# moxime/joint-vae

Measured on NVIDIA B200. Metric: train_images_per_sec, higher is better.
Workload: dtype bf16

## Files before the change

joint-vae_b200/csrc/conv.cu:

```cuda
#include "tc_common.cuh"
#include <vector>
#include <algorithm>
#include <stdlib.h>

namespace jvae {

constexpr int CONV_THREADS = 192;
constexpr int CONV_MAX_TAPS = 64;
static thread_local int g_last_conv_kernel = 0;

struct ConvParams {
  int N, Hq, Wq;
  int TW, TH, NB;
  int tiles_x, tiles_y, tiles_n, num_tiles, n_tiles_n;
  int Cblk, nCk, ntaps;
  int in_stride;
  short dy[CONV_MAX_TAPS], dx[CONV_MAX_TAPS];
  int BN;
  int Ho, Wo, Cout, ldc;
  int out_sy, out_sx, out_oy, out_ox;
  int act;
  int out_f32;
  const float* bias;
  __nv_bfloat16* out;
// ... 747 lines not shown
        int m = tile;
        const int tx = m % p.tiles_x; m /= p.tiles_x;
        const int ty = m % p.tiles_y; m /= p.tiles_y;
        const int n0 = m * p.NB;
        for (int t = 0; t < ntap; ++t, ++it) {
          const int s = it % p.stages;
          const uint32_t ph = (it / p.stages) & 1;
          mbar_wait(&empty_bar[s], ph ^ 1);
          uint8_t* sa = smem + (size_t)s * p.stage_bytes;
          mbar_arrive_expect_tx(&full_bar[s], p.tx_bytes);
          tma_load_4d(sa, &tmap_dy, &full_bar[s], cy0, tx * p.TW, ty * p.TH, n0);
          tma_load_4d(sa + p.a_bytes, &tmap_x, &full_bar[s], cx0, tx * p.TW * p.in_stride + p.dx[tap_lo + t],
                      ty * p.TH * p.in_stride + p.dy[tap_lo + t], n0);
        }
      }
    }
  } else if (warp == 1) {
    if (elect_one()) {
      const uint32_t idesc = make_idesc_bf16(64, p.Cblk_x, true, true);
      const uint32_t swz_y = (p.Cblk_y == 64) ? SWZ_128B : (p.Cblk_y == 32 ? SWZ_64B : SWZ_32B);
      const uint32_t swz_x = (p.Cblk_x == 64) ? SWZ_128B : (p.Cblk_x == 32 ? SWZ_64B : SWZ_32B);
      const uint32_t row_y = (uint32_t)p.Cblk_y * 2u, row_x = (uint32_t)p.Cblk_x * 2u;
      uint32_t it = 0;
      bool first_tile = true;
      for (int tile = blockIdx.x; tile < p.num_tiles; tile += gridDim.x) {
        for (int t = 0; t < ntap; ++t, ++it) {
          const int s = it % p.stages;
          const uint32_t ph = (it / p.stages) & 1;
          mbar_wait(&full_bar[s], ph);
          tc_fence_after();
          const uint32_t sa = smem_u32(smem + (size_t)s * p.stage_bytes);
          const uint64_t a_desc = make_smem_desc(sa, 8 * row_y, 8 * row_y, swz_y);
          const uint64_t b_desc = make_smem_desc(sa + p.a_bytes, 8 * row_x, 8 * row_x, swz_x);
          const uint32_t d_tmem = tmem_base + (uint32_t)(t * p.Cblk_x);
#pragma unroll
          for (int k = 0; k < 8; ++k)
            umma_bf16(d_tmem, a_desc + (uint64_t)((16 * row_y * k) >> 4), b_desc + (uint64_t)((16 * row_x * k) >> 4), idesc,
                      (!first_tile || k != 0));
          umma_commit(&empty_bar[s]);
        }
        first_tile = false;
      }
      umma_commit(done_bar);
    }
  } else {
    const int q = warp & 3;
    mbar_wait(done_bar, 0);
    tc_fence_after();
    const bool has_work = blockIdx.x < p.num_tiles;
    for (int t = 0; t < ntap && has_work; ++t) {
      for (int c0 = 0; c0 < p.Cblk_x; c0 += 16) {
        uint32_t r[16];
        tmem_ld_32x16(tmem_base + ((uint32_t)(q * 32) << 16) + (uint32_t)(t * p.Cblk_x + c0), r);
        tmem_ld_wait();
        const int row = q * 16 + lane;
        if (lane < 16 && row < M_real) {
          float* o = p.dw + (size_t)(tap_lo + t) * p.dw_ld_tap + (size_t)(cy0 + row) * p.dw_ld_co + (size_t)(cx0 + c0) * p.dw_ld_cx;
#pragma unroll
          for (int j = 0; j < 16; ++j)
            if (c0 + j < N_real) atomicAdd(o + (size_t)j * p.dw_ld_cx, __uint_as_float(r[j]));
        }
      }
    }
  }
  tc_fence_before();
  __syncthreads();
  if (warp == 1) tmem_dealloc_dyn(tmem_base, p.tmem_cols);
}

constexpr int WH_MAX_GROUPS = 64;
struct WHaloParams {
  int N, Hq, Wq;
  int NBt, HHs, HWp, MT, strips_x, num_boxes;
  int RT, blocks_y;
  uint32_t g_img_bytes;
  int Cblk_g, Cblk_x, ncx, Cg, Cx;
  int ngroups, groups_per_cta;
  int dymin, dxmin, ey;
  int in_stride, nplanes;
  short plane_ry[4], plane_rx[4];
  uint32_t plane_bytes;
  uint32_t grp_off16[WH_MAX_GROUPS];
  unsigned char grp_ntap[WH_MAX_GROUPS];
  unsigned char grp_nv[WH_MAX_GROUPS];
  uint32_t grp_boff16[WH_MAX_GROUPS];
  uint32_t grp_idesc[WH_MAX_GROUPS];
  unsigned short grp_col[WH_MAX_GROUPS];
  short grp_tap[WH_MAX_GROUPS][8][8];
  uint32_t g_gap_bytes;
  float* dw;
  int dw_ld_tap, dw_ld_co, dw_ld_cx;
  uint32_t x_stage_bytes, stage_bytes, x_box_bytes, g_box_bytes, tmem_cols;
  int stages;
};

__global__ void __launch_bounds__(CONV_THREADS, 1)
conv_wgrad_halo_kernel(const __grid_constant__ CUtensorMap tmap_g, const __grid_constant__ CUtensorMap tmap_x,
                       const __grid_constant__ WHaloParams p) {
  extern __shared__ uint8_t smem_raw[];
  uint8_t* smem = reinterpret_cast<uint8_t*>((reinterpret_cast<uintptr_t>(smem_raw) + 1023) & ~(uintptr_t)1023);
  uint64_t* full_bar = reinterpret_cast<uint64_t*>(smem + (size_t)p.stages * p.stage_bytes);
  uint64_t* empty_bar = full_bar + 8;
  uint64_t* done_bar = empty_bar + 8;
  uint32_t* tmem_slot = reinterpret_cast<uint32_t*>(done_bar + 1);
  const int warp = threadIdx.x >> 5, lane = threadIdx.x & 31;
  const int g_lo = (int)blockIdx.y * p.groups_per_cta;
  const int ng = min(p.groups_per_cta, p.ngroups - g_lo);
  const int cg0 = ((int)blockIdx.z / p.ncx) * p.Cblk_g, cx0 = ((int)blockIdx.z % p.ncx) * p.Cblk_x;
  const uint32_t rbx = (uint32_t)p.Cblk_x * 2u, rbg = (uint32_t)p.Cblk_g * 2u;

  for (uint32_t i = threadIdx.x; i < (uint32_t)p.stages * p.stage_bytes / 16u; i += CONV_THREADS)
    reinterpret_cast<uint4*>(smem)[i] = make_uint4(0u, 0u, 0u, 0u);
  if (warp == 0 && lane == 0) {
    tma_prefetch_desc(&tmap_g);
    tma_prefetch_desc(&tmap_x);
    for (int s = 0; s < 8; ++s) { mbar_init(&full_bar[s], 1); mbar_init(&empty_bar[s], 1); }
    mbar_init(done_bar, 1);
    fence_barrier_init();
  }
  fence_proxy_async();
  if (warp == 1) tmem_alloc_dyn(tmem_slot, p.tmem_cols);
  tc_fence_before();
  __syncthreads();
  tc_fence_after();
  const uint32_t tmem_base = *tmem_slot;

  if (warp == 0) {
    if (elect_one()) {
      uint32_t s = 0, ph = 0;
      for (int box = blockIdx.x; box < p.num_boxes; box += gridDim.x) {
        int m = box;
        const int sx = m % p.strips_x; m /= p.strips_x;
        const int by = m % p.blocks_y; const int nb = m / p.blocks_y;
        mbar_wait(&empty_bar[s], ph ^ 1);
        uint8_t* st = smem + (size_t)s * p.stage_bytes;
        mbar_arrive_expect_tx(&full_bar[s], p.x_box_bytes + p.g_box_bytes);
        for (int pl = 0; pl < p.nplanes; ++pl)
          tma_load_4d(st + (size_t)pl * p.plane_bytes, &tmap_x, &full_bar[s], cx0, p.in_stride * (sx * 8 + p.dxmin) + p.plane_rx[pl],
                      p.in_stride * (by * p.RT + p.dymin) + p.plane_ry[pl], nb * p.NBt);
        if (p.blocks_y == 1) {
          tma_load_4d(st + p.x_stage_bytes + p.g_gap_bytes, &tmap_g, &full_bar[s], cg0, sx * 8, 0, nb * p.NBt);
        } else {
          for (int i = 0; i < p.NBt; ++i)
            tma_load_4d(st + p.x_stage_bytes + p.g_gap_bytes + (size_t)i * p.HHs * 8u * rbg, &tmap_g, &full_bar[s], cg0, sx * 8,
                        by * p.RT, nb * p.NBt + i);
        }
        if (++s == (uint32_t)p.stages) { s = 0; ph ^= 1; }
      }
    }
  } else if (warp == 1) {
    if (elect_one()) {
      const uint32_t swx = (p.Cblk_x == 64) ? SWZ_128B : (p.Cblk_x == 32 ? SWZ_64B : SWZ_32B);
      const uint32_t swg = (p.Cblk_g == 64) ? SWZ_128B : (p.Cblk_g == 32 ? SWZ_64B : SWZ_32B);
      const uint32_t a_hi = (((uint32_t)p.HWp * rbx >> 4) & 0x3fffu) | (1u << 14) | (swx << 29);
      const uint32_t b_hi = (((8u * rbg) >> 4) & 0x3fffu) | (1u << 14) | (swg << 29);
      const uint32_t a_lbo = ((rbx >> 4) & 0x3fffu) << 16, b_lbo = (((8u * rbg) >> 4) & 0x3fffu) << 16;
      const uint32_t ak16 = (2u * (uint32_t)p.HWp * rbx) >> 4, bk16 = (16u * rbg) >> 4;
      const uint32_t am16 = (16u * (uint32_t)p.HWp * rbx) >> 4, bm16 = (128u * rbg) >> 4;
      const uint32_t ey_slots16 = ((uint32_t)p.ey * 8u * rbg) >> 4;
      uint32_t s = 0, ph = 0, first = 0;
      for (int box = blockIdx.x; box < p.num_boxes; box += gridDim.x) {
        mbar_wait(&full_bar[s], ph);
        tc_fence_after();
        const uint32_t sx_ = smem_u32(smem + (size_t)s * p.stage_bytes);
        const uint32_t a_lo0 = ((sx_ >> 4) & 0x3fffu) | a_lbo;
        const uint32_t b_lo0 = ((((sx_ + p.x_stage_bytes + p.g_gap_bytes) >> 4) - ey_slots16) & 0x3fffu) | b_lbo;
        for (int m = 0; m < p.MT; ++m) {
          const uint32_t b_lo = b_lo0 + (uint32_t)m * bm16;
          for (int g = 0; g < ng; ++g) {
            const uint32_t a_lo = a_lo0 + (uint32_t)m * am16 + p.grp_off16[g_lo + g];
            const uint32_t bg_lo = b_lo + p.grp_boff16[g_lo + g];
            const uint32_t idesc = p.grp_idesc[g_lo + g];
            const uint32_t d = tmem_base + (uint32_t)p.grp_col[g_lo + g];
#pragma unroll
            for (int k = 0; k < 8; ++k)
              umma_bf16(d, desc64(a_hi, a_lo + (uint32_t)k * ak16), desc64(b_hi, bg_lo + (uint32_t)k * bk16), idesc,
                        k == 0 ? first : 1u);
          }
          first = 1;
        }
        umma_commit(&empty_bar[s]);
        if (++s == (uint32_t)p.stages) { s = 0; ph ^= 1; }
      }
      umma_commit(done_bar);
    }
  } else {
    const int q = warp & 3;
    mbar_wait(done_bar, 0);
    tc_fence_after();
    const bool has_work = (int)blockIdx.x < p.num_boxes;
    const int Ng = min(p.Cblk_g, p.Cg - cg0), Nx = min(p.Cblk_x, p.Cx - cx0);
    for (int g = 0; g < ng && has_work; ++g) {
      const int ntap = p.grp_ntap[g_lo + g];
      const bool m128 = ntap * p.Cblk_x > 64;
      const int row = m128 ? q * 32 + lane : q * 16 + lane;
      const bool row_ok = m128 || lane < 16;
      const int j = row / p.Cblk_x, cx = row - j * p.Cblk_x;
      const bool live = row_ok && j < ntap && cx < Nx;
      const int nv = p.grp_nv[g_lo + g];
      for (int jv = 0; jv < nv; ++jv) {
        const int t = live ? p.grp_tap[g_lo + g][jv][j] : 0;
        for (int c0 = 0; c0 < p.Cblk_g; c0 += 16) {
          uint32_t r[16];
          tmem_ld_32x16(tmem_base + ((uint32_t)(q * 32) << 16) + (uint32_t)(p.grp_col[g_lo + g] + jv * p.Cblk_g + c0), r);
          tmem_ld_wait();
          if (live) {
            float* o = p.dw + (size_t)t * p.dw_ld_tap + (size_t)(cg0 + c0) * p.dw_ld_co + (size_t)(cx0 + cx) * p.dw_ld_cx;
#pragma unroll
            for (int i = 0; i < 16; ++i)
              if (c0 + i < Ng) atomicAdd(o + (size_t)i * p.dw_ld_co, __uint_as_float(r[i]));
          }
        }
      }
    }
  }
  tc_fence_before();
  __syncthreads();
  if (warp == 1) tmem_dealloc_dyn(tmem_base, p.tmem_cols);
}

static int pow2_floor(int v) { int p = 1; while (p * 2 <= v) p *= 2; return p; }
static int pow2_ceil(int v) { int p = 1; while (p < v) p *= 2; return p; }

static void tile_shape(int Hq, int Wq, int* TW, int* TH, int* NB) {
  int tw = pow2_floor(Wq); if (tw > 128) tw = 128;
  if (tw < Wq && tw * 2 <= 128 && (tw * 2 - Wq) * 4 <= Wq) tw *= 2;
  int th = pow2_ceil(Hq); if (th > 128 / tw) th = 128 / tw;
  *TW = tw; *TH = th; *NB = 128 / (tw * th);
}

static int cblk_of(int C) { return C > 32 ? 64 : (C > 16 ? 32 : 16); }

static int act_tmap(CUtensorMap* t, const void* base, int N, int H, int W, int C, int ldc, int Cblk, int TW, int TH, int NB,
                    int stride) {
  uint64_t dims[4] = {(uint64_t)C, (uint64_t)W, (uint64_t)H, (uint64_t)N};
  uint64_t strides[3] = {(uint64_t)ldc * 2, (uint64_t)W * ldc * 2, (uint64_t)H * W * ldc * 2};
  uint32_t box[4] = {(uint32_t)Cblk, (uint32_t)(TW * stride), (uint32_t)(TH * stride), (uint32_t)NB};
  uint32_t es[4] = {1, (uint32_t)stride, (uint32_t)stride, 1};
  return make_tmap_bf16(t, base, 4, dims, strides, box, es, Cblk * 2);
}

struct PhaseSpec { int n; const int16_t* ntaps; const int16_t* oy; const int16_t* ox; };

static int try_launch_halo(const void* in, int N, int H, int W, int Cin, int ld_in, const void* wmat, int Cout_pad, int ldw,
                           int ntaps, const int16_t* tap_dy, const int16_t* tap_dx, int in_stride, int Hq, int Wq, void* out,
                           int Ho, int Wo, int Cout, int ld_out, int out_sy, int out_sx, int out_oy, int out_ox,
                           const float* bias, int act, double* stats, const jvae_bn_reduce* bn, int* bn_fused,
                           cudaStream_t stream, const PhaseSpec* phs = nullptr, HaloParams* plan_out = nullptr,
                           int force_cblk = 0, double* score_out = nullptr) {
  if (Wq < 6) return 1;
  const bool wide = Cin > 64 || Cout_pad > 64;
  if (phs && (wide || in_stride != 1 || phs->n < 2 || phs->n > 4 || bn)) return 1;
  if (wide) {
    const bool wide_on = getenv("JVAE_CONV_WIDE") && atoi(getenv("JVAE_CONV_WIDE")) != 0;
    if (!wide_on || (Cout_pad > 64 && (Cout_pad % 64) != 0) || bn) return 1;
  }
  if (bn && !(out_sy == 1 && out_sx == 1 && out_oy == 0 && out_ox == 0 && Ho == Hq && Wo == Wq)) {
    bn = nullptr; stats = nullptr;
  }
  if (!phs && !wide && force_cblk == 0 && Cin > 32 && !(getenv("JVAE_CONV_KSPLIT") && atoi(getenv("JVAE_CONV_KSPLIT")) == 0)) {
    HaloParams pa, pb;
    double sa = 0.0, sb = 0.0;
    const int ra = try_launch_halo(in, N, H, W, Cin, ld_in, wmat, Cout_pad, ldw, ntaps, tap_dy, tap_dx, in_stride, Hq, Wq, out, Ho, Wo,
                                   Cout, ld_out, out_sy, out_sx, out_oy, out_ox, bias, act, stats, bn, nullptr, stream, nullptr, &pa, 64, &sa);
    const int rb2 = try_launch_halo(in, N, H, W, Cin, ld_in, wmat, Cout_pad, ldw, ntaps, tap_dy, tap_dx, in_stride, Hq, Wq, out, Ho, Wo,
                                    Cout, ld_out, out_sy, out_sx, out_oy, out_ox, bias, act, stats, bn, nullptr, stream, nullptr, &pb, 32, &sb);
    if (ra < 0) return ra;
    const int pick = (rb2 == 0 && (ra != 0 || sb > 1.15 * sa)) ? 32 : 64;
    if (score_out) *score_out = pick == 32 ? sb : sa;
    return try_launch_halo(in, N, H, W, Cin, ld_in, wmat, Cout_pad, ldw, ntaps, tap_dy, tap_dx, in_stride, Hq, Wq, out, Ho, Wo, Cout,
                           ld_out, out_sy, out_sx, out_oy, out_ox, bias, act, stats, bn, bn_fused, stream, nullptr, plan_out, pick, nullptr);
  }
  HaloParams p;
  memset(&p, 0, sizeof(p));
  p.PH = 1;
  const int st = in_stride;
  int tey[CONV_MAX_TAPS], tex[CONV_MAX_TAPS], tpl[CONV_MAX_TAPS];
  int dymin = 1 << 20, dymax = -(1 << 20), dxmin = 1 << 20, dxmax = -(1 << 20);
  p.in_stride = st; p.nplanes = 0;
  for (int t = 0; t < ntaps; ++t) {
    p.dy[t] = tap_dy[t]; p.dx[t] = tap_dx[t];
    const int ry = ((tap_dy[t] % st) + st) % st, rx = ((tap_dx[t] % st) + st) % st;
    tey[t] = (tap_dy[t] - ry) / st; tex[t] = (tap_dx[t] - rx) / st;
    int pl = -1;
    for (int i = 0; i < p.nplanes; ++i)
      if (p.plane_ry[i] == ry && p.plane_rx[i] == rx) pl = i;
    if (pl < 0) { pl = p.nplanes++; p.plane_ry[pl] = (short)ry; p.plane_rx[pl] = (short)rx; }
    tpl[t] = pl;
    dymin = min(dymin, tey[t]); dymax = max(dymax, tey[t]);
// ... 194 lines not shown
      p.ck[nck].y = ((uint32_t)(col_base[ci] + q.e_hi - (u - j0)) * p.w_tap_bytes) >> 4;
      p.ck[nck].z = make_idesc_bf16(128, (j1 - j0 + 1) * p.BN, false, false);
      p.ck[nck].w = (uint32_t)(j0 * p.BN) | (fresh ? 0x80000000u : 0u);
      ++nck;
    };
    std::vector<int> fresh_u;
    for (int jn = 0; jn < p.G;) {
      const int u = jn + cols[0].e_hi;
      fresh_u.push_back(u);
      jn = min(p.G - 1, u - cols[0].e_lo) + 1;
    }
    for (int u : fresh_u) add_chunk(0, u, 1);
    for (size_t ci = 0; ci < cols.size(); ++ci)
      for (int u = cols[ci].e_lo; u <= cols[ci].e_hi + p.G - 1; ++u) {
        if (ci == 0 && std::find(fresh_u.begin(), fresh_u.end(), u) != fresh_u.end()) continue;
        if (nck >= HALO_MAX_CK) return 1;
        add_chunk(ci, u, 0);
      }
    p.nck = nck;
    if ((((uint32_t)pos * p.w_tap_bytes) >> 4) > 0xffffu) return 1;
  }
  p.box_bytes = (uint32_t)p.nplanes * (uint32_t)(p.NBt * p.HHs) * p.HWp * rb;
  {
    const uint32_t bud = budget + (p.G > 1 ? 20u * 1024u : 0u);
    p.stages = (int)((bud - p.w_bytes - stats_bytes - 1792u - (uint32_t)(p.MT * p.G * p.PH) * 128u) / p.stage_bytes);
  }
  if (p.stages > 4) p.stages = 4;
  if (p.stages < 2) return 1;
  p.acc_stride = (uint32_t)(p.MT * p.G * p.PH * p.BN);
  p.tmem_cols = (uint32_t)pow2_ceil(2 * p.acc_stride < 32 ? 32 : 2 * p.acc_stride);
  p.strips_x = (Wq + 7) / 8; p.blocks_y = (Hq + p.RT - 1) / p.RT; p.blocks_n = (N + p.NBt - 1) / p.NBt;
  p.num_boxes = p.strips_x * p.blocks_y * p.blocks_n;
  p.Ho = Ho; p.Wo = Wo; p.Cout = Cout; p.ldc = ld_out;
  p.out_sy = out_sy; p.out_sx = out_sx; p.out_oy = out_oy; p.out_ox = out_ox;
  p.act = act & 0xff; p.out_f32 = (act & JVAE_OUT_F32) ? 1 : 0;
  p.bias = bias; p.out = reinterpret_cast<__nv_bfloat16*>(out); p.stats = stats; p.cout_pad = Cout_pad;
  if (plan_out) { *plan_out = p; return JVAE_OK; }
  CUtensorMap tin, tw;
  if (bn) {
    p.bn_y = reinterpret_cast<const __nv_bfloat16*>(bn->y); p.bn_ld = bn->ld_y; p.bn_save = bn->save_mean_rstd;
    p.bn_gamma = bn->gamma; p.bn_beta = bn->beta; p.bn_act = bn->act;
    if ((bn->ld_y % 8) != 0) { set_error("jvae_conv_gather_gemm_bn: bn.ld_y must be a multiple of 8"); return JVAE_ERR_INVALID; }
    if (!stats) { set_error("jvae_conv_gather_gemm_bn: the sums need the stats buffer"); return JVAE_ERR_INVALID; }
  }
  {
    uint64_t dims[4] = {(uint64_t)Cin, (uint64_t)W, (uint64_t)H, (uint64_t)N};
    uint64_t strides[3] = {(uint64_t)ld_in * 2, (uint64_t)W * ld_in * 2, (uint64_t)H * W * ld_in * 2};
    uint32_t box[4] = {(uint32_t)p.Cblk, (uint32_t)(p.HWp * st), (uint32_t)(p.HHs * st), (uint32_t)p.NBt};
    uint32_t es[4] = {1u, (uint32_t)st, (uint32_t)st, 1u};
    if (box[1] > 256 || box[2] > 256) return 1;
    int rc = make_tmap_bf16(&tin, in, 4, dims, strides, box, es, p.Cblk * 2);
    if (rc) return rc;
    const int Ktot = ntaps * p.nkc * p.Cblk;
    uint64_t wd[2] = {(uint64_t)Ktot, (uint64_t)Cout_pad};
    uint64_t ws[1] = {(uint64_t)ldw * 2};
    uint32_t wbox[2] = {(uint32_t)p.Cblk, (uint32_t)p.BN};
    if (ldw < Ktot) { set_error("jvae_conv_gather_gemm: weight matrix row shorter than taps*Cblk"); return JVAE_ERR_INVALID; }
    rc = make_tmap_bf16(&tw, wmat, 2, wd, ws, wbox, nullptr, p.Cblk * 2);
    if (rc) return rc;
  }
  const size_t tab_bytes = (size_t)p.MT * p.G * p.PH * 16 * sizeof(int2);
  const size_t smem = (size_t)p.stages * p.stage_bytes + p.w_bytes + 512 + stats_bytes +
                      256 + 1024 + 1024 + tab_bytes;
  if (smem > 227u * 1024u) return 1;
  static bool attr = false;
  if (!attr) {
    JVAE_CUDA(cudaFuncSetAttribute(conv_halo_kernel, cudaFuncAttributeMaxDynamicSharedMemorySize, 227 * 1024));
    attr = true;
  }
  int grid = p.num_boxes * p.n_tiles_n < sm_count() ? p.num_boxes * p.n_tiles_n : (sm_count() / p.n_tiles_n) * p.n_tiles_n;
  if (grid < p.n_tiles_n) return 1;
  void* prof = prof_begin(JVAE_PROF_CONV_HALO, stream);
  conv_halo_kernel<<<grid, HALO_THREADS, smem, stream>>>(tin, tw, p);
  prof_end(prof, stream);
  JVAE_LAUNCH_CHECK();
  g_last_conv_kernel = JVAE_KERNEL_CONV_HALO;
  if (bn && bn_fused) *bn_fused = 1;
  return JVAE_OK;
}

static int try_launch_wgrad_halo(const void* g, int N, int Hq, int Wq, int Cg, int ld_g, const void* x, int H, int W, int Cx,
                                 int ld_x, int ntaps, const int16_t* tap_dy, const int16_t* tap_dx, int in_stride, float* dw,
                                 int dw_ld_tap, int dw_ld_co, int dw_ld_cx, cudaStream_t stream, const int* tap_ids = nullptr,
                                 bool dry_run = false, WHaloParams* plan_out = nullptr) {
  if (Wq < 6) return 1;
  WHaloParams p;
  memset(&p, 0, sizeof(p));
  const int st = in_stride;
  std::vector<int> tey(ntaps), tex(ntaps), tpl(ntaps);
  int dymin = 1 << 20, dymax = -(1 << 20), dxmin = 1 << 20, dxmax = -(1 << 20);
  p.in_stride = st; p.nplanes = 0;
  for (int t = 0; t < ntaps; ++t) {
    const int ry = ((tap_dy[t] % st) + st) % st, rx = ((tap_dx[t] % st) + st) % st;
    tey[t] = (tap_dy[t] - ry) / st; tex[t] = (tap_dx[t] - rx) / st;
    int pl = -1;
    for (int i = 0; i < p.nplanes; ++i)
      if (p.plane_ry[i] == ry && p.plane_rx[i] == rx) pl = i;
    if (pl < 0) { pl = p.nplanes++; p.plane_ry[pl] = (short)ry; p.plane_rx[pl] = (short)rx; }
    tpl[t] = pl;
    dymin = min(dymin, tey[t]); dymax = max(dymax, tey[t]);
    dxmin = min(dxmin, tex[t]); dxmax = max(dxmax, tex[t]);
  }
  const int ey = dymax - dymin, ex = dxmax - dxmin;
  if (ey > 16 || ex > 16) return 1;
  p.N = N; p.Hq = Hq; p.Wq = Wq; p.dymin = dymin; p.dxmin = dxmin;
  p.Cg = Cg; p.Cx = Cx;
  p.Cblk_g = cblk_of(Cg > 64 ? 64 : Cg); p.Cblk_x = cblk_of(Cx > 64 ? 64 : Cx);
  const int ncg = (Cg + p.Cblk_g - 1) / p.Cblk_g;
  p.ncx = (Cx + p.Cblk_x - 1) / p.Cblk_x;
  const uint32_t rbx = (uint32_t)p.Cblk_x * 2u, rbg = (uint32_t)p.Cblk_g * 2u;
  p.RT = Hq <= 32 ? Hq : 32; p.blocks_y = (Hq + p.RT - 1) / p.RT;
  p.HWp = 8 + ex; p.HHs = p.RT + ey;
  const int tpm = 128 / p.Cblk_x;
  p.ey = ey;
  std::vector<int> tap_at((size_t)(ey + 1) * (ex + 1), -1);
  bool want = (cblk_of(Cg > 64 ? 64 : Cg) == 32 && ey + 1 >= 4) || (ey + 1 == 3 && Hq * Wq <= 64 && Cg >= 128);
  if (const char* e = getenv("JVAE_WGRAD_VSTACK")) want = atoi(e) != 0;
  bool full = want && st == 1 && p.nplanes == 1 && ntaps == (ey + 1) * (ex + 1);
  for (int t = 0; t < ntaps && full; ++t) {
    int& slot = tap_at[(size_t)(tey[t] - dymin) * (ex + 1) + (tex[t] - dxmin)];
    if (slot >= 0) full = false;
    slot = t;
  }
  int ngr = 0;
  std::vector<int> grp_first;
  const uint32_t gslot16 = (8u * rbg) >> 4;
  const int E = ey;
  if (full) {
    int nvmax = min(ey + 1, 256 / p.Cblk_g);
    if (const char* e = getenv("JVAE_WGRAD_NVMAX")) nvmax = max(1, min(nvmax, atoi(e)));
    const int nsets = (ey + 1 + nvmax - 1) / nvmax;
    for (int x0 = 0; x0 <= ex; x0 += min(tpm, 8)) {
      const int n = min(min(tpm, 8), ex + 1 - x0);
      for (int vs = 0, v0 = 0; vs < nsets; ++vs) {
        const int nv = (ey + 1 - v0 + (nsets - vs) - 1) / (nsets - vs);
        if (ngr >= WH_MAX_GROUPS) return 1;
        p.grp_ntap[ngr] = (unsigned char)n;
        p.grp_nv[ngr] = (unsigned char)nv;
        p.grp_off16[ngr] = ((uint32_t)x0 * rbx) >> 4;
        p.grp_boff16[ngr] = (uint32_t)v0 * gslot16;
        for (int jv = 0; jv < nv; ++jv)
          for (int j = 0; j < n; ++j) {
            const int t = tap_at[(size_t)(ey - v0 - jv) * (ex + 1) + (x0 + j)];
            p.grp_tap[ngr][jv][j] = (short)(tap_ids ? tap_ids[t] : t);
          }
        ++ngr;
        v0 += nv;
      }
    }
  } else {
    std::vector<int> order(ntaps);
    for (int t = 0; t < ntaps; ++t) order[t] = t;
    std::sort(order.begin(), order.end(), [&](int a, int b) {
      if (tpl[a] != tpl[b]) return tpl[a] < tpl[b];
      return tey[a] != tey[b] ? tey[a] < tey[b] : tex[a] < tex[b];
    });
    for (int i = 0; i < ntaps;) {
      if (ngr >= WH_MAX_GROUPS) return 1;
      int n = 1;
      while (i + n < ntaps && n < tpm && n < 8 && tpl[order[i + n]] == tpl[order[i]] && tey[order[i + n]] == tey[order[i]] &&
             tex[order[i + n]] == tex[order[i]] + n)
        ++n;
      p.grp_ntap[ngr] = (unsigned char)n;
      p.grp_nv[ngr] = 1;
      p.grp_boff16[ngr] = (uint32_t)E * gslot16;
      grp_first.push_back(order[i]);
      for (int j = 0; j < n; ++j) p.grp_tap[ngr][0][j] = (short)(tap_ids ? tap_ids[order[i + j]] : order[i + j]);
      ++ngr;
      i += n;
    }
  }
  p.ngroups = ngr;
  int wmax = 0;
  for (int gi = 0; gi < ngr; ++gi) {
    const int M = ((int)p.grp_ntap[gi] * p.Cblk_x > 64) ? 128 : 64;
    p.grp_idesc[gi] = make_idesc_bf16(M, (int)p.grp_nv[gi] * p.Cblk_g, true, true);
    wmax = max(wmax, (int)p.grp_nv[gi] * p.Cblk_g);
  }
  p.groups_per_cta = 512 / wmax;
  if (p.groups_per_cta > ngr) p.groups_per_cta = ngr;
  const int ysplit = (ngr + p.groups_per_cta - 1) / p.groups_per_cta;
  p.groups_per_cta = (ngr + ysplit - 1) / ysplit;
  int cols_max = 0;
  for (int gi = 0; gi < ngr; gi += p.groups_per_cta) {
    int col = 0;
    for (int k = gi; k < min(ngr, gi + p.groups_per_cta); ++k) { p.grp_col[k] = (unsigned short)col; col += (int)p.grp_nv[k] * p.Cblk_g; }
    cols_max = max(cols_max, col);
  }
  p.tmem_cols = (uint32_t)pow2_ceil(cols_max < 32 ? 32 : cols_max);
  p.g_gap_bytes = ((uint32_t)E * 8u * rbg + 1023u) & ~1023u;
  p.ey = E;
  const uint32_t budget = 200u * 1024u;
  double best = 0.0;
  for (int nbt = 1; nbt <= 16 && nbt <= N; ++nbt) {
    const int S = nbt * p.HHs, MT = full ? (S + 15) / 16 : (S - ey + 15) / 16;
    const uint32_t plane = ((uint32_t)(16 * MT + ey + 1) * p.HWp * rbx + 1023u) & ~1023u;
    const uint32_t xs = plane * (uint32_t)p.nplanes;
    const uint32_t gs = p.g_gap_bytes + (((uint32_t)(16 * MT > S ? 16 * MT : S) * 8u * rbg + 1023u) & ~1023u);
    if (2u * (xs + gs) + 1024u > budget) break;
    if (nbt * p.HHs > 256) break;
    const double eff = (double)(nbt * p.RT) / (16.0 * MT);
    if (eff > best + 0.02) {
      best = eff; p.NBt = nbt; p.MT = MT; p.x_stage_bytes = xs; p.stage_bytes = xs + gs; p.plane_bytes = plane;
    }
  }
  if (best <= 0.0) return 1;
  if ((size_t)p.stage_bytes >= (1u << 18)) return 1;
  for (int gi = 0; gi < ngr && !full; ++gi) {
    const int t0 = grp_first[gi];
    p.grp_off16[gi] = ((uint32_t)tpl[t0] * p.plane_bytes + (uint32_t)((tey[t0] - dymin) * p.HWp + (tex[t0] - dxmin)) * rbx) >> 4;
  }
  p.x_box_bytes = (uint32_t)p.nplanes * (uint32_t)(p.NBt * p.HHs) * p.HWp * rbx;
  p.g_box_bytes = (uint32_t)(p.NBt * (p.blocks_y == 1 ? p.HHs : p.RT)) * 8u * rbg;
  p.stages = (int)((budget - 1024u) / p.stage_bytes);
  if (p.stages > 6) p.stages = 6;
  if (p.stages < 2) return 1;
  p.strips_x = (Wq + 7) / 8;
  p.num_boxes = p.strips_x * p.blocks_y * ((N + p.NBt - 1) / p.NBt);
  p.dw = dw; p.dw_ld_tap = dw_ld_tap; p.dw_ld_co = dw_ld_co; p.dw_ld_cx = dw_ld_cx;
  if (plan_out) *plan_out = p;
  if (dry_run) return JVAE_OK;
  CUtensorMap tg, tx;
  {
    uint64_t dg[4] = {(uint64_t)Cg, (uint64_t)Wq, (uint64_t)Hq, (uint64_t)N};
    uint64_t sg[3] = {(uint64_t)ld_g * 2, (uint64_t)Wq * ld_g * 2, (uint64_t)Hq * Wq * ld_g * 2};
    uint32_t bg[4] = {(uint32_t)p.Cblk_g, 8u, (uint32_t)(p.blocks_y == 1 ? p.HHs : p.RT), (uint32_t)(p.blocks_y == 1 ? p.NBt : 1)};
    int rc = make_tmap_bf16(&tg, g, 4, dg, sg, bg, nullptr, p.Cblk_g * 2);
    if (rc) return rc;
    uint64_t dx[4] = {(uint64_t)Cx, (uint64_t)W, (uint64_t)H, (uint64_t)N};
    uint64_t sx[3] = {(uint64_t)ld_x * 2, (uint64_t)W * ld_x * 2, (uint64_t)H * W * ld_x * 2};
    uint32_t bx[4] = {(uint32_t)p.Cblk_x, (uint32_t)(p.HWp * st), (uint32_t)(p.HHs * st), (uint32_t)p.NBt};
    uint32_t esx[4] = {1u, (uint32_t)st, (uint32_t)st, 1u};
    if (bx[1] > 256 || bx[2] > 256) return 1;
    rc = make_tmap_bf16(&tx, x, 4, dx, sx, bx, esx, p.Cblk_x * 2);
    if (rc) return rc;
  }
  const int nz = ncg * p.ncx;
  if (nz > 65535) return 1;
  int gx = (sm_count() + ysplit * nz - 1) / (ysplit * nz);
  if (gx < 1) gx = 1;
  if (gx > p.num_boxes) gx = p.num_boxes;
  const size_t smem = (size_t)p.stages * p.stage_bytes + 256 + 1024;
  static bool attr = false;
  if (!attr) {
    JVAE_CUDA(cudaFuncSetAttribute(conv_wgrad_halo_kernel, cudaFuncAttributeMaxDynamicSharedMemorySize, 227 * 1024));
    attr = true;
  }
  void* prof = prof_begin(JVAE_PROF_WGRAD_HALO, stream);
  conv_wgrad_halo_kernel<<<dim3(gx, ysplit, nz), CONV_THREADS, smem, stream>>>(tg, tx, p);
  prof_end(prof, stream);
  JVAE_LAUNCH_CHECK();
  g_last_conv_kernel = JVAE_KERNEL_WGRAD_HALO;
  return JVAE_OK;
}


static void wgrad_plan_emulate(const WHaloParams& p, const float* g, int ld_g, const float* x, int H, int W, int ld_x, float* dw) {
  const int ncg = (p.Cg + p.Cblk_g - 1) / p.Cblk_g;
  const size_t plane_rows = p.plane_bytes / ((size_t)p.Cblk_x * 2u);
  const size_t x_rows = plane_rows * p.nplanes;
  const int gap_slots = (int)(p.g_gap_bytes / (8u * (uint32_t)p.Cblk_g * 2u));
  const size_t g_slots = (size_t)gap_slots + (size_t)((p.stage_bytes - p.x_stage_bytes - p.g_gap_bytes) / (8u * (uint32_t)p.Cblk_g * 2u));
  std::vector<float> sx(x_rows * p.Cblk_x), sg(g_slots * 8 * p.Cblk_g);
  const float qnan = nanf("");
  for (int zg = 0; zg < ncg; ++zg)
    for (int zx = 0; zx < p.ncx; ++zx) {
      const int cg0 = zg * p.Cblk_g, cx0 = zx * p.Cblk_x;
      std::vector<double> D((size_t)p.ngroups * 128 * 8 * p.Cblk_g, 0.0);
      for (int box = 0; box < p.num_boxes; ++box) {
        int m0 = box;
        const int bx = m0 % p.strips_x; m0 /= p.strips_x;
        const int by = m0 % p.blocks_y; const int nb = m0 / p.blocks_y;
        std::fill(sx.begin(), sx.end(), 0.f);
        std::fill(sg.begin(), sg.end(), 0.f);
        for (int pl = 0; pl < p.nplanes; ++pl)
          for (int i = 0; i < p.NBt; ++i)
            for (int yy = 0; yy < p.HHs; ++yy)
              for (int xx = 0; xx < p.HWp; ++xx) {
                const size_t row = (size_t)pl * plane_rows + (size_t)(i * p.HHs + yy) * p.HWp + xx;
                const int n = nb * p.NBt + i;
                const int iy = p.in_stride * (by * p.RT + p.dymin + yy) + p.plane_ry[pl], ix = p.in_stride * (bx * 8 + p.dxmin + xx) + p.plane_rx[pl];
                for (int c = 0; c < p.Cblk_x; ++c) {
                  const bool in = n < p.N && iy >= 0 && iy < H && ix >= 0 && ix < W && cx0 + c < p.Cx;
                  if (row < x_rows) sx[row * p.Cblk_x + c] = in ? x[(((size_t)n * H + iy) * W + ix) * ld_x + cx0 + c] : 0.f;
                }
              }
        for (int i = 0; i < p.NBt; ++i)
          for (int yy = 0; yy < (p.blocks_y == 1 ? p.HHs : p.RT); ++yy)
            for (int px = 0; px < 8; ++px) {
              const size_t slot = (size_t)gap_slots + (size_t)i * p.HHs + yy;
              const int n = nb * p.NBt + i, gy = by * p.RT + yy, gx = bx * 8 + px;
              for (int c = 0; c < p.Cblk_g; ++c) {
                const bool in = n < p.N && gy < p.Hq && gx < p.Wq && cg0 + c < p.Cg;
                if (slot < g_slots) sg[(slot * 8 + px) * p.Cblk_g + c] = in ? g[(((size_t)n * p.Hq + gy) * p.Wq + gx) * ld_g + cg0 + c] : 0.f;
              }
            }
        auto xa = [&](long long row, int c) { return row >= 0 && (size_t)row < x_rows ? sx[(size_t)row * p.Cblk_x + c] : qnan; };
        auto ga = [&](long long slot, int px, int c) { return slot >= 0 && (size_t)slot < g_slots ? sg[((size_t)slot * 8 + px) * p.Cblk_g + c] : qnan; };
        for (int m = 0; m < p.MT; ++m)
          for (int gi = 0; gi < p.ngroups; ++gi) {
            const long long a_rows = (long long)p.grp_off16[gi] * 16 / (p.Cblk_x * 2);
            const long long b_slots = (long long)gap_slots - p.ey + (long long)p.grp_boff16[gi] * 16 / (8 * p.Cblk_g * 2);
            const int ntap = p.grp_ntap[gi], nv = p.grp_nv[gi];
            for (int k = 0; k < 8; ++k)
              for (int kk = 0; kk < 16; ++kk) {
                const long long s = 16 * m + 2 * k + (kk >> 3);
                for (int j = 0; j < ntap; ++j)
                  for (int cx = 0; cx < p.Cblk_x; ++cx) {
                    const float a = xa(a_rows + s * p.HWp + (kk & 7) + j, cx);
                    if (a == 0.f) continue;
                    for (int jv = 0; jv < nv; ++jv)
                      for (int cg = 0; cg < p.Cblk_g; ++cg)
                        D[(((size_t)gi * 128 + (size_t)j * p.Cblk_x + cx) * 8 + jv) * p.Cblk_g + cg] += (double)a * (double)ga(b_slots + s + jv, kk & 7, cg);
                  }
              }
          }
      }
      for (int gi = 0; gi < p.ngroups; ++gi)
        for (int j = 0; j < p.grp_ntap[gi]; ++j)
          for (int jv = 0; jv < p.grp_nv[gi]; ++jv) {
            const int t = p.grp_tap[gi][jv][j];
            for (int cx = 0; cx < p.Cblk_x && cx0 + cx < p.Cx; ++cx)
              for (int cg = 0; cg < p.Cblk_g && cg0 + cg < p.Cg; ++cg)
                dw[(size_t)t * p.dw_ld_tap + (size_t)(cg0 + cg) * p.dw_ld_co + (size_t)(cx0 + cx) * p.dw_ld_cx] +=
                    (float)D[(((size_t)gi * 128 + (size_t)j * p.Cblk_x + cx) * 8 + jv) * p.Cblk_g + cg];
          }
    }
}

}

using namespace jvae;

extern "C" {

int jvae_conv_gather_gemm(const void* in, int N, int H, int W, int Cin, int ld_in, const void* wmat, int Cout_pad, int ldw,
                          int ntaps, const int16_t* tap_dy, const int16_t* tap_dx, int in_stride, int Hq, int Wq,
                          void* out, int Ho, int Wo, int Cout, int ld_out, int out_sy, int out_sx, int out_oy, int out_ox,
                          const float* bias, int act, double* stats, void* stream) {
  return jvae_conv_gather_gemm_bn(in, N, H, W, Cin, ld_in, wmat, Cout_pad, ldw, ntaps, tap_dy, tap_dx, in_stride, Hq, Wq, out, Ho,
                                  Wo, Cout, ld_out, out_sy, out_sx, out_oy, out_ox, bias, act, stats, nullptr, nullptr, stream);
}

int jvae_conv_gather_gemm_bn(const void* in, int N, int H, int W, int Cin, int ld_in, const void* wmat, int Cout_pad, int ldw,
                             int ntaps, const int16_t* tap_dy, const int16_t* tap_dx, int in_stride, int Hq, int Wq,
                             void* out, int Ho, int Wo, int Cout, int ld_out, int out_sy, int out_sx, int out_oy, int out_ox,
                             const float* bias, int act, double* stats, const jvae_bn_reduce* bn, int* bn_fused, void* stream) {
  JVAE_CHECK_ARG(in && wmat && out && tap_dy && tap_dx, "null pointer");
  JVAE_CHECK_ARG(!bn || (bn->y && bn->save_mean_rstd && stats && bn->ld_y >= Cout), "bn reduce needs y, save_mean_rstd and the sums buffer");
  if (bn_fused) *bn_fused = 0;
  JVAE_CHECK_ARG(ntaps >= 1 && ntaps <= CONV_MAX_TAPS, "1..64 taps");
  JVAE_CHECK_ARG((ld_in % 8) == 0 && (ldw % 8) == 0, "input / weight channel strides must be multiples of 8");
  JVAE_CHECK_ARG(ld_out >= Cout, "ld_out < Cout");
  JVAE_CHECK_ARG((Cout_pad % 16) == 0 && Cout_pad >= 16 && Cout_pad >= Cout, "Cout_pad must be a multiple of 16, >= Cout");
  JVAE_CHECK_ARG(!stats || Cout_pad <= 2048, "statistics epilogue supports up to 2048 channels");
  JVAE_CHECK_ARG(in_stride == 1 || in_stride == 2, "input stride 1 or 2");
  JVAE_CHECK_ARG((((uintptr_t)in | (uintptr_t)wmat | (uintptr_t)out) & 15) == 0, "16-byte alignment");
  static const bool force_v1 = getenv("JVAE_CONV_V1") != nullptr;
  if (!force_v1) {
    const int rc = try_launch_halo(in, N, H, W, Cin, ld_in, wmat, Cout_pad, ldw, ntaps, tap_dy, tap_dx, in_stride, Hq, Wq, out,
                                   Ho, Wo, Cout, ld_out, out_sy, out_sx, out_oy, out_ox, bias, act, stats, bn, bn_fused,
                                   (cudaStream_t)stream);
    if (rc <= 0) return rc;
  }
  if (bn) stats = nullptr;
  ConvParams p;
  memset(&p, 0, sizeof(p));
  p.N = N; p.Hq = Hq; p.Wq = Wq;
  tile_shape(Hq, Wq, &p.TW, &p.TH, &p.NB);
  p.tiles_x = (Wq + p.TW - 1) / p.TW; p.tiles_y = (Hq + p.TH - 1) / p.TH; p.tiles_n = (N + p.NB - 1) / p.NB;
  p.BN = Cout_pad > 256 ? 256 : Cout_pad;
  if (Cout_pad > 256) JVAE_CHECK_ARG((Cout_pad % 256) == 0, "Cout_pad > 256 must be a multiple of 256");
  static const bool narrow = !(getenv("JVAE_CONV_NARROW") && atoi(getenv("JVAE_CONV_NARROW")) == 0);
  while (narrow && p.BN > 64 && (p.BN % 32) == 0 && 2 * p.tiles_x * p.tiles_y * p.tiles_n * (Cout_pad / p.BN) <= sm_count()) p.BN /= 2;
  p.n_tiles_n = Cout_pad / p.BN;
  p.num_tiles = p.tiles_x * p.tiles_y * p.tiles_n * p.n_tiles_n;
  p.Cblk = cblk_of(Cin); p.nCk = (Cin + p.Cblk - 1) / p.Cblk; p.ntaps = ntaps; p.in_stride = in_stride;
  for (int t = 0; t < ntaps; ++t) { p.dy[t] = tap_dy[t]; p.dx[t] = tap_dx[t]; }
  p.Ho = Ho; p.Wo = Wo; p.Cout = Cout; p.ldc = ld_out;
  p.out_sy = out_sy; p.out_sx = out_sx; p.out_oy = out_oy; p.out_ox = out_ox;
  p.act = act & 0xff; p.out_f32 = (act & JVAE_OUT_F32) ? 1 : 0;
  p.bias = bias; p.out = reinterpret_cast<__nv_bfloat16*>(out);
  p.stats = stats; p.cout_pad = Cout_pad;
  const uint32_t stats_bytes = stats ? 2u * (uint32_t)Cout_pad * 8u : 0u;
  p.a_bytes = 128u * p.Cblk * 2u;
  p.tx_bytes = p.a_bytes + (uint32_t)p.BN * p.Cblk * 2u;
  p.stage_bytes = (p.tx_bytes + 1023u) & ~1023u;
  p.stages = (int)((200u * 1024u - stats_bytes) / p.stage_bytes);
  if (p.stages > 12) p.stages = 12;
  JVAE_CHECK_ARG(p.stages >= 2, "tile too large for shared memory");
  p.tmem_cols = (uint32_t)pow2_ceil(2 * p.BN < 32 ? 32 : 2 * p.BN);
  CUtensorMap tin, tw;
  int rc = act_tmap(&tin, in, N, H, W, Cin, ld_in, p.Cblk, p.TW, p.TH, p.NB, in_stride);
  if (rc) return rc;
  {
    const int Ktot = ntaps * p.nCk * p.Cblk;
    uint64_t dims[2] = {(uint64_t)Ktot, (uint64_t)Cout_pad};
    uint64_t strides[1] = {(uint64_t)ldw * 2};
    uint32_t box[2] = {(uint32_t)p.Cblk, (uint32_t)p.BN};
    JVAE_CHECK_ARG(ldw >= Ktot, "weight matrix row shorter than taps*chunks*Cblk");
    rc = make_tmap_bf16(&tw, wmat, 2, dims, strides, box, nullptr, p.Cblk * 2);
    if (rc) return rc;
  }
  const size_t smem = (size_t)p.stages * p.stage_bytes + 256 + stats_bytes + 1024;
// ... 549 lines not shown
```

Baseline: 45440.

## Pack wgrad halo taps into horizontal/vertical UMMA groups via per-group A leading offset

Adds a packed tap-grouping planner for the weight-gradient halo kernel. Taps in each plane can now be grouped along rows or columns, with a per-group A-descriptor leading byte offset, and vertical-tap groups use the N dimension. A cost model picks the cheaper covering, and the packing is kept only if it is clearly cheaper than the old grouping. The aim is to cut the number of UMMA groups and issued MMAs per box, at the cost of larger x stages, extra descriptor data in params, and a recursive fallback when the packed plan does not fit.

```diff
diff --git a/joint-vae_b200/csrc/conv.cu b/joint-vae_b200/csrc/conv.cu
--- a/joint-vae_b200/csrc/conv.cu
+++ b/joint-vae_b200/csrc/conv.cu
@@ -853,6 +853,8 @@
   uint32_t plane_bytes;
   uint32_t grp_off16[WH_MAX_GROUPS];
   unsigned char grp_ntap[WH_MAX_GROUPS];
+  unsigned short grp_alb16[WH_MAX_GROUPS];
+  unsigned char grp_m128[WH_MAX_GROUPS];
   unsigned char grp_nv[WH_MAX_GROUPS];
   uint32_t grp_boff16[WH_MAX_GROUPS];
   uint32_t grp_idesc[WH_MAX_GROUPS];
@@ -925,7 +927,7 @@
       const uint32_t swg = (p.Cblk_g == 64) ? SWZ_128B : (p.Cblk_g == 32 ? SWZ_64B : SWZ_32B);
       const uint32_t a_hi = (((uint32_t)p.HWp * rbx >> 4) & 0x3fffu) | (1u << 14) | (swx << 29);
       const uint32_t b_hi = (((8u * rbg) >> 4) & 0x3fffu) | (1u << 14) | (swg << 29);
-      const uint32_t a_lbo = ((rbx >> 4) & 0x3fffu) << 16, b_lbo = (((8u * rbg) >> 4) & 0x3fffu) << 16;
+      const uint32_t b_lbo = (((8u * rbg) >> 4) & 0x3fffu) << 16;
       const uint32_t ak16 = (2u * (uint32_t)p.HWp * rbx) >> 4, bk16 = (16u * rbg) >> 4;
       const uint32_t am16 = (16u * (uint32_t)p.HWp * rbx) >> 4, bm16 = (128u * rbg) >> 4;
       const uint32_t ey_slots16 = ((uint32_t)p.ey * 8u * rbg) >> 4;
@@ -934,12 +936,12 @@
         mbar_wait(&full_bar[s], ph);
         tc_fence_after();
         const uint32_t sx_ = smem_u32(smem + (size_t)s * p.stage_bytes);
-        const uint32_t a_lo0 = ((sx_ >> 4) & 0x3fffu) | a_lbo;
+        const uint32_t a_lo0 = (sx_ >> 4) & 0x3fffu;
         const uint32_t b_lo0 = ((((sx_ + p.x_stage_bytes + p.g_gap_bytes) >> 4) - ey_slots16) & 0x3fffu) | b_lbo;
         for (int m = 0; m < p.MT; ++m) {
           const uint32_t b_lo = b_lo0 + (uint32_t)m * bm16;
           for (int g = 0; g < ng; ++g) {
-            const uint32_t a_lo = a_lo0 + (uint32_t)m * am16 + p.grp_off16[g_lo + g];
+            const uint32_t a_lo = (a_lo0 + (uint32_t)m * am16 + p.grp_off16[g_lo + g]) | (((uint32_t)p.grp_alb16[g_lo + g] & 0x3fffu) << 16);
             const uint32_t bg_lo = b_lo + p.grp_boff16[g_lo + g];
             const uint32_t idesc = p.grp_idesc[g_lo + g];
             const uint32_t d = tmem_base + (uint32_t)p.grp_col[g_lo + g];
@@ -963,7 +965,7 @@
     const int Ng = min(p.Cblk_g, p.Cg - cg0), Nx = min(p.Cblk_x, p.Cx - cx0);
     for (int g = 0; g < ng && has_work; ++g) {
       const int ntap = p.grp_ntap[g_lo + g];
-      const bool m128 = ntap * p.Cblk_x > 64;
+      const bool m128 = p.grp_m128[g_lo + g] != 0;
       const int row = m128 ? q * 32 + lane : q * 16 + lane;
       const bool row_ok = m128 || lane < 16;
       const int j = row / p.Cblk_x, cx = row - j * p.Cblk_x;
@@ -975,7 +977,7 @@
           uint32_t r[16];
           tmem_ld_32x16(tmem_base + ((uint32_t)(q * 32) << 16) + (uint32_t)(p.grp_col[g_lo + g] + jv * p.Cblk_g + c0), r);
           tmem_ld_wait();
-          if (live) {
+          if (live && t >= 0) {
             float* o = p.dw + (size_t)t * p.dw_ld_tap + (size_t)(cg0 + c0) * p.dw_ld_co + (size_t)(cx0 + cx) * p.dw_ld_cx;
 #pragma unroll
             for (int i = 0; i < 16; ++i)
@@ -1336,7 +1338,7 @@
 static int try_launch_wgrad_halo(const void* g, int N, int Hq, int Wq, int Cg, int ld_g, const void* x, int H, int W, int Cx,
                                  int ld_x, int ntaps, const int16_t* tap_dy, const int16_t* tap_dx, int in_stride, float* dw,
                                  int dw_ld_tap, int dw_ld_co, int dw_ld_cx, cudaStream_t stream, const int* tap_ids = nullptr,
-                                 bool dry_run = false, WHaloParams* plan_out = nullptr) {
+                                 bool dry_run = false, WHaloParams* plan_out = nullptr, bool packed = true) {
   if (Wq < 6) return 1;
   WHaloParams p;
   memset(&p, 0, sizeof(p));
@@ -1380,7 +1382,120 @@
   std::vector<int> grp_first;
   const uint32_t gslot16 = (8u * rbg) >> 4;
   const int E = ey;
-  if (full) {
+  struct WGrp { int pl, vert, nm, r0, c0, nv, boff; };
+  std::vector<WGrp> pk;
+  std::vector<int> pk_at;
+  int pk_bmin = 0, pk_vreach = 0;
+  {
+    const char* pe = getenv("JVAE_WGRAD_PACK");
+    const char* fc = getenv("JVAE_WGRAD_COVER");
+    const bool on = packed && !(pe && atoi(pe) == 0) && !(fc && (strlen(fc) != 2 || !strchr("1s", fc[0]) || !strchr("hvd", fc[1])));
+    int rlo[4], rhi[4], clo[4], chi[4], cnt[4] = {0, 0, 0, 0};
+    for (int i = 0; i < 4; ++i) { rlo[i] = clo[i] = 1 << 20; rhi[i] = chi[i] = -1; }
+    pk_at.assign((size_t)p.nplanes * (ey + 1) * (ex + 1), -1);
+    bool rect = on;
+    for (int t = 0; t < ntaps && rect; ++t) {
+      const int pl = tpl[t], y = tey[t] - dymin, x = tex[t] - dxmin;
+      rlo[pl] = min(rlo[pl], y); rhi[pl] = max(rhi[pl], y); clo[pl] = min(clo[pl], x); chi[pl] = max(chi[pl], x); ++cnt[pl];
+      int& slot = pk_at[((size_t)pl * (ey + 1) + y) * (ex + 1) + x];
+      if (slot >= 0) rect = false;
+      slot = t;
+    }
+    for (int pl = 0; pl < p.nplanes && rect; ++pl) rect = cnt[pl] == (rhi[pl] - rlo[pl] + 1) * (chi[pl] - clo[pl] + 1);
+    int nvcap = 256 / p.Cblk_g;
+    if (const char* e = getenv("JVAE_WGRAD_NVMAX")) nvcap = max(1, min(nvcap, atoi(e)));
+    const int w = min(tpm, 8);
+    auto gen = [&](int pl, int body, int tail, std::vector<WGrp>& out) {
+      const int R = rhi[pl] - rlo[pl] + 1, C = chi[pl] - clo[pl] + 1;
+      const int Cb = (tail == 0 || R == 1) ? C : (C / w) * w;
+      for (int x0 = 0; x0 < Cb; x0 += w) {
+        const int n = min(w, Cb - x0);
+        if (!body || R == 1) {
+          for (int y = rlo[pl]; y <= rhi[pl]; ++y) out.push_back({pl, 0, n, y, clo[pl] + x0, 1, E});
+        } else {
+          const int nvm = min(R, nvcap), nsets = (R + nvm - 1) / nvm;
+          for (int vs = 0, v0 = 0; vs < nsets; ++vs) {
+            const int nv = (R - v0 + (nsets - vs) - 1) / (nsets - vs);
+            out.push_back({pl, 0, n, rlo[pl], clo[pl] + x0, nv, E - (R - 1) + v0});
+            v0 += nv;
+          }
+        }
+      }
+      for (int c = Cb; c < C; ++c) {
+        const int m = min(w, R), nv = R - m + 1;
+        if (tail == 2 && nv <= nvcap) {
+          out.push_back({pl, 1, m, rlo[pl], clo[pl] + c, nv, E - (nv - 1)});
+        } else {
+          for (int y0 = rlo[pl]; y0 <= rhi[pl]; y0 += w) out.push_back({pl, 1, min(w, rhi[pl] - y0 + 1), y0, clo[pl] + c, 1, E});
+        }
+      }
+    };
+    const int S1 = p.HHs * max(1, min(N, 128 / p.HHs));
+    auto cost = [&](const std::vector<WGrp>& v) {
+      double c = 0.0;
+      int b0 = 0;
+      for (const WGrp& q : v) {
+        c += (50.0 + 0.4 * q.nv * p.Cblk_g) * (q.nv > 1 ? 1.9 : 1.0);
+        b0 = min(b0, q.boff - E);
+      }
+      return c * (double)((S1 - ey - b0 + 15) / 16);
+    };
+    if (rect) {
+      double c_new = 0.0, c_old = 0.0;
+      for (int pl = 0; pl < p.nplanes; ++pl) {
+        std::vector<WGrp> best, cand;
+        gen(pl, full ? 1 : 0, 0, best);
+        c_old += cost(best);
+        if (fc) {
+          best.clear();
+          gen(pl, fc[0] == 's', fc[1] == 'h' ? 0 : (fc[1] == 'v' ? 1 : 2), best);
+        } else {
+          for (int tail = 1; tail < 3; ++tail) {
+            cand.clear();
+            gen(pl, full ? 1 : 0, tail, cand);
+            if (cost(cand) < cost(best)) best = cand;
+          }
+        }
+        c_new += cost(best);
+        pk.insert(pk.end(), best.begin(), best.end());
+      }
+      if (!fc && c_new > 0.9 * c_old) pk.clear();
+    }
+  }
+  if (!pk.empty()) {
+    std::vector<char> covered(ntaps, 0);
+    bool ok = (int)pk.size() <= WH_MAX_GROUPS;
+    pk_bmin = 0; pk_vreach = 0;
+    for (int gi = 0; gi < (int)pk.size() && ok; ++gi) {
+      const WGrp& q = pk[gi];
+      const bool m128 = q.nm * p.Cblk_x > 64;
+      if (q.nm > 8 || q.nv > 8) { ok = false; break; }
+      p.grp_ntap[gi] = (unsigned char)q.nm;
+      p.grp_nv[gi] = (unsigned char)q.nv;
+      p.grp_m128[gi] = m128 ? 1 : 0;
+      p.grp_alb16[gi] = (unsigned short)(((uint32_t)(q.vert ? p.HWp : 1) * rbx) >> 4);
+      p.grp_boff16[gi] = (uint32_t)q.boff * gslot16;
+      for (int jv = 0; jv < 8; ++jv)
+        for (int j = 0; j < 8; ++j) p.grp_tap[gi][jv][j] = -1;
+      for (int jv = 0; jv < q.nv; ++jv)
+        for (int j = 0; j < q.nm; ++j) {
+          const int b = q.boff - E + jv, y = q.r0 + (q.vert ? j : 0) - b, x = q.c0 + (q.vert ? 0 : j);
+          if (b > 0 || b < -E) ok = false;
+          int t = (y >= 0 && y <= ey && x >= 0 && x <= ex) ? pk_at[((size_t)q.pl * (ey + 1) + y) * (ex + 1) + x] : -1;
+          if (t >= 0 && covered[t]) t = -1;
+          if (t < 0) continue;
+          covered[t] = 1;
+          pk_bmin = min(pk_bmin, b);
+          p.grp_tap[gi][jv][j] = (short)(tap_ids ? tap_ids[t] : t);
+        }
+      if (q.vert) pk_vreach = max(pk_vreach, q.r0 + (m128 ? 128 : 64) / p.Cblk_x);
+    }
+    for (int t = 0; t < ntaps && ok; ++t) ok = covered[t] != 0;
+    if (ok) ngr = (int)pk.size();
+    else pk.clear();
+  }
+  if (!pk.empty()) {
+  } else if (full) {
     int nvmax = min(ey + 1, 256 / p.Cblk_g);
     if (const char* e = getenv("JVAE_WGRAD_NVMAX")) nvmax = max(1, min(nvmax, atoi(e)));
     const int nsets = (ey + 1 + nvmax - 1) / nvmax;
@@ -1427,7 +1542,11 @@
   p.ngroups = ngr;
   int wmax = 0;
   for (int gi = 0; gi < ngr; ++gi) {
-    const int M = ((int)p.grp_ntap[gi] * p.Cblk_x > 64) ? 128 : 64;
+    if (pk.empty()) {
+      p.grp_m128[gi] = (int)p.grp_ntap[gi] * p.Cblk_x > 64 ? 1 : 0;
+      p.grp_alb16[gi] = (unsigned short)(rbx >> 4);
+    }
+    const int M = p.grp_m128[gi] ? 128 : 64;
     p.grp_idesc[gi] = make_idesc_bf16(M, (int)p.grp_nv[gi] * p.Cblk_g, true, true);
     wmax = max(wmax, (int)p.grp_nv[gi] * p.Cblk_g);
   }
@@ -1446,9 +1565,11 @@
   p.ey = E;
   const uint32_t budget = 200u * 1024u;
   double best = 0.0;
+  const int bmin = !pk.empty() ? pk_bmin : (full ? -E : 0);
+  const int xtail = max(ey + 1, pk_vreach);
   for (int nbt = 1; nbt <= 16 && nbt <= N; ++nbt) {
-    const int S = nbt * p.HHs, MT = full ? (S + 15) / 16 : (S - ey + 15) / 16;
-    const uint32_t plane = ((uint32_t)(16 * MT + ey + 1) * p.HWp * rbx + 1023u) & ~1023u;
+    const int S = nbt * p.HHs, MT = (S - ey - bmin + 15) / 16;
+    const uint32_t plane = ((uint32_t)(16 * MT + xtail) * p.HWp * rbx + 1023u) & ~1023u;
     const uint32_t xs = plane * (uint32_t)p.nplanes;
     const uint32_t gs = p.g_gap_bytes + (((uint32_t)(16 * MT > S ? 16 * MT : S) * 8u * rbg + 1023u) & ~1023u);
     if (2u * (xs + gs) + 1024u > budget) break;
@@ -1458,9 +1579,14 @@
       best = eff; p.NBt = nbt; p.MT = MT; p.x_stage_bytes = xs; p.stage_bytes = xs + gs; p.plane_bytes = plane;
     }
   }
-  if (best <= 0.0) return 1;
-  if ((size_t)p.stage_bytes >= (1u << 18)) return 1;
-  for (int gi = 0; gi < ngr && !full; ++gi) {
+  auto unpacked = [&]() {
+    return try_launch_wgrad_halo(g, N, Hq, Wq, Cg, ld_g, x, H, W, Cx, ld_x, ntaps, tap_dy, tap_dx, in_stride, dw, dw_ld_tap,
+                                 dw_ld_co, dw_ld_cx, stream, tap_ids, dry_run, plan_out, false);
+  };
+  if (best <= 0.0 || (size_t)p.stage_bytes >= (1u << 18) || (budget - 1024u) / p.stage_bytes < 2u) return pk.empty() ? 1 : unpacked();
+  for (int gi = 0; gi < ngr && !pk.empty(); ++gi)
+    p.grp_off16[gi] = ((uint32_t)pk[gi].pl * p.plane_bytes + (uint32_t)(pk[gi].r0 * p.HWp + pk[gi].c0) * rbx) >> 4;
+  for (int gi = 0; gi < ngr && pk.empty() && !full; ++gi) {
     const int t0 = grp_first[gi];
     p.grp_off16[gi] = ((uint32_t)tpl[t0] * p.plane_bytes + (uint32_t)((tey[t0] - dymin) * p.HWp + (tex[t0] - dxmin)) * rbx) >> 4;
   }
@@ -1555,13 +1681,14 @@
           for (int gi = 0; gi < p.ngroups; ++gi) {
             const long long a_rows = (long long)p.grp_off16[gi] * 16 / (p.Cblk_x * 2);
             const long long b_slots = (long long)gap_slots - p.ey + (long long)p.grp_boff16[gi] * 16 / (8 * p.Cblk_g * 2);
+            const long long a_lbo_rows = (long long)p.grp_alb16[gi] * 16 / (p.Cblk_x * 2);
             const int ntap = p.grp_ntap[gi], nv = p.grp_nv[gi];
             for (int k = 0; k < 8; ++k)
               for (int kk = 0; kk < 16; ++kk) {
                 const long long s = 16 * m + 2 * k + (kk >> 3);
                 for (int j = 0; j < ntap; ++j)
                   for (int cx = 0; cx < p.Cblk_x; ++cx) {
-                    const float a = xa(a_rows + s * p.HWp + (kk & 7) + j, cx);
+                    const float a = xa(a_rows + s * p.HWp + (kk & 7) + j * a_lbo_rows, cx);
                     if (a == 0.f) continue;
                     for (int jv = 0; jv < nv; ++jv)
                       for (int cg = 0; cg < p.Cblk_g; ++cg)
@@ -1574,6 +1701,7 @@
         for (int j = 0; j < p.grp_ntap[gi]; ++j)
           for (int jv = 0; jv < p.grp_nv[gi]; ++jv) {
             const int t = p.grp_tap[gi][jv][j];
+            if (t < 0) continue;
             for (int cx = 0; cx < p.Cblk_x && cx0 + cx < p.Cx; ++cx)
               for (int cg = 0; cg < p.Cblk_g && cg0 + cg < p.Cg; ++cg)
                 dw[(size_t)t * p.dw_ld_tap + (size_t)(cg0 + cg) * p.dw_ld_co + (size_t)(cx0 + cx) * p.dw_ld_cx] +=
```

Measured after the change: 45590 (median of 6 runs). About the same (+0.3%).
